# aslpavel/svgrasterize.py

Measured on AMD Instinct MI355X. Metric: Mpixels/sec AA coverage+composite (path-pixels/s; whole step: flatten+binning+coverage+composite; planned replay -- a frame with new geometry: value_replan), higher is better.
Workload: dtype f64 arithmetic, f32 RGBA store; 1 GPU; synthetic 4096 random closed cubic paths @ 4096x4096 (SURVEY 8d generator, splitmix64 0x5F3759DF); edges=783607

## Files before the change

### svgrasterize.py_amd/csrc/svgr_core.h

```cpp
#pragma once
#include <math.h>
#include <stdint.h>

#if defined(__HIPCC__)
#define SVGR_HD __host__ __device__ __forceinline__
#define SVGR_UNROLL _Pragma("unroll")
#else
#define SVGR_HD static inline
#define SVGR_UNROLL
#endif

namespace svgr {

constexpr int kMaxFlattenDepth = 40;
constexpr double kZeroCut = 1e-6;

SVGR_HD void xform_point(const double* m6, double p0, double p1, double& o0, double& o1) {
    o0 = fma(p1, m6[1], p0 * m6[0]) + m6[2];
    o1 = fma(p1, m6[4], p0 * m6[3]) + m6[5];
}

SVGR_HD double dot4(double w0, double w1, double w2, double w3, double x0, double x1, double x2, double x3) {
    return fma(w0, x0, w2 * x2) + fma(w1, x1, w3 * x3);
}
// ... 262 lines not shown
            if (!put(x1i - 1, d * (1.0 - a2 - am))) return;
        }
        put(x1i, d * am);
    }
}

struct RowPieces {
    int x0i, n;
    double v[5];
};

SVGR_HD RowPieces row_record(double x, double x_next, double d) {
    RowPieces r;
    double x0 = x < x_next ? x : x_next;
    double x1 = x < x_next ? x_next : x;
    double x0_floor = floor(x0);
    r.x0i = clamp_to_int(x0_floor);
    double x1_ceil = ceil(x1);
    int x1i = clamp_to_int(x1_ceil);
    r.v[2] = r.v[3] = r.v[4] = 0.0;
    if (x1i <= r.x0i + 1) {
        double xmf = 0.5 * (x + x_next) - x0_floor;
        r.n = 1;
        r.v[0] = d * (1 - xmf);
        r.v[1] = d * xmf;
    } else {
        double s = 1 / (x1 - x0);
        double x0f = x0 - x0_floor;
        double x1f = x1 - x1_ceil + 1.0;
        double o = 1 - x0f;
        double a0 = 0.5 * s * (o * o);
        double am = 0.5 * s * (x1f * x1f);
        r.n = x1i - r.x0i;
        r.v[0] = d * a0;
        r.v[4] = d * am;
        if (r.n == 2) {
            r.v[1] = d * (1.0 - a0 - am);
        } else {
            double a1 = s * (1.5 - x0f);
            r.v[1] = d * (a1 - a0);
            r.v[2] = d * s;
            double a2 = a1 + (double)(x1i - r.x0i - 3) * s;
            r.v[3] = d * (1.0 - a2 - am);
        }
    }
    return r;
}

SVGR_HD int band_room(double x_in, double x_out, int nr, int cols, int px, int& lo, int& hi) {
    double xlo = x_in < x_out ? x_in : x_out, xhi = x_in < x_out ? x_out : x_in;
    xlo -= 1e-9 * (1.0 + fabs(xlo));
    xhi += 1e-9 * (1.0 + fabs(xhi));
    lo = clamp_to_int(floor(xlo));
    hi = clamp_to_int(floor(xhi));
    const int lo_c = lo > -1 ? lo : -1;
    int hi_c = hi > -1 ? hi : -1;
    hi_c = hi_c < cols ? hi_c : cols;
    const int nc = hi_c - lo_c, fold = lo < 0 ? 3 * nr : 0;
    int room = 2 * nr + nc;
    room = room < 6 * nr + nc / px + 1 ? room : 6 * nr + nc / px + 1;
    return (room < 13 * nr ? room : 13 * nr) + fold;
}

template <class Put>
SVGR_HD void apply_record(int x0i, int n, const double* v, Put&& put) {
    if (!put(x0i, v[0])) return;
    if (!put(x0i + 1, v[1])) return;
    if (n >= 3) {
        for (int xi = x0i + 2; xi < x0i + n - 1; ++xi)
            if (!put(xi, v[2])) return;
        if (!put(x0i + n - 1, v[3])) return;
    }
    if (n >= 2) put(x0i + n, v[4]);
}

SVGR_HD void row_span(double x, double x_next, int& lo, int& hi) {
    double x0 = x < x_next ? x : x_next;
    double x1 = x < x_next ? x_next : x;
    lo = clamp_to_int(floor(x0));
    int x1i = clamp_to_int(ceil(x1));
    hi = (x1i <= lo + 1) ? lo + 1 : x1i;
}

SVGR_HD double fill_nonzero_raw(double s) {
    double m = fabs(s);
    return m > 1.0 ? 1.0 : m;
}
SVGR_HD double fill_nonzero(double s) {
    double m = fill_nonzero_raw(s);
    return m < kZeroCut ? 0.0 : m;
}
SVGR_HD double fill_evenodd_raw(double s) {
    double a = s + 1.0;
    double r = a - 2.0 * floor(a * 0.5);
    return fabs(r - 1.0);
}
SVGR_HD double fill_evenodd(double s) {
    double a = s + 1.0;
    double r = a - 2.0 * floor(a * 0.5);
    double m = fabs(r - 1.0);
    return m < kZeroCut ? 0.0 : m;
}
SVGR_HD double fill_rule(double s, int rule) { return rule ? fill_evenodd(s) : fill_nonzero(s); }

SVGR_HD void over_px(double* dst, double s0, double s1, double s2, double s3) {
    double k = 1 - s3;
    dst[0] = s0 + dst[0] * k;
    dst[1] = s1 + dst[1] * k;
    dst[2] = s2 + dst[2] * k;
    dst[3] = s3 + dst[3] * k;
}

SVGR_HD void over_px_fma(double* dst, double s0, double s1, double s2, double s3) {
    double k = 1 - s3;
    dst[0] = fma(dst[0], k, s0);
    dst[1] = fma(dst[1], k, s1);
    dst[2] = fma(dst[2], k, s2);
    dst[3] = fma(dst[3], k, s3);
}

constexpr int kTurbBSize = 0x100, kTurbBM = 0xff, kTurbN = 0x1000;
constexpr int kTurbLattice = kTurbBSize + kTurbBSize + 2;
constexpr int kTurbMaxOctaves = 32;
constexpr int64_t kTurbM = 2147483647, kTurbA = 16807, kTurbQ = 127773, kTurbR = 2836;

SVGR_HD int64_t turb_setup_seed(int64_t s) {
    if (s <= 0) s = -(s % (kTurbM - 1)) + 1;
    if (s > kTurbM - 1) s = kTurbM - 1;
    return s;
}

SVGR_HD int64_t turb_random(int64_t s) {
    int64_t r = kTurbA * (s % kTurbQ) - kTurbR * (s / kTurbQ);
    if (r <= 0) r += kTurbM;
    return r;
}

SVGR_HD void turb_init(int64_t seed, int* sel, double* grad) {
    int64_t s = turb_setup_seed(seed);
    for (int k = 0; k < 4; ++k) {
        for (int i = 0; i < kTurbBSize; ++i) {
            sel[i] = i;
            for (int j = 0; j < 2; ++j) {
                s = turb_random(s);
                grad[(i * 4 + k) * 2 + j] = (double)(s % (2 * kTurbBSize) - kTurbBSize) / kTurbBSize;
            }
            double* g = grad + (i * 4 + k) * 2;
            const double len = sqrt(g[0] * g[0] + g[1] * g[1]);
            if (len > 0.0) {
                g[0] = g[0] / len;
                g[1] = g[1] / len;
            }
        }
    }
    for (int i = kTurbBSize - 1; i > 0; --i) {
        const int t = sel[i];
        s = turb_random(s);
        const int j = (int)(s % kTurbBSize);
        sel[i] = sel[j];
        sel[j] = t;
    }
    for (int i = 0; i < kTurbBSize + 2; ++i) {
        sel[kTurbBSize + i] = sel[i];
        for (int q = 0; q < 8; ++q) grad[(kTurbBSize + i) * 8 + q] = grad[i * 8 + q];
    }
}
// ... 482 lines not shown
```

### svgrasterize.py_amd/csrc/svgr_hip.hip

```cpp
#include <hip/hip_runtime.h>

#include <algorithm>
#include <atomic>
#include <cstdarg>
#include <cstddef>
#include <cmath>
#include <cstdio>
#include <cstring>
#include <ctime>
#include <initializer_list>
#include <new>
#include <string>
#include <type_traits>
#include <vector>
#include <memory>
#include <unordered_map>
#include <utility>

#include "../../include/svgr.h"
#include "svgr_core.h"

using namespace svgr;

static std::atomic<unsigned long long> g_n_launches{0};
#define SVGR_LAUNCH(...) do { g_n_launches.fetch_add(1, std::memory_order_relaxed); hipLaunchKernelGGL(__VA_ARGS__); } while (0)

constexpr int TR = 16;
constexpr int PX = 8;
constexpr int CH = 8;
constexpr int TC = CH * PX;
constexpr int NT = TR * CH;
constexpr int CHUNK_STRIDE = PX + 2;
constexpr int ROW_STRIDE = CH * CHUNK_STRIDE;
constexpr int DELTA_BYTES = TR * ROW_STRIDE * 8;
static_assert(DELTA_BYTES < (1 << 16), "a TileAdd carries its byte offset in 16 bits");
static_assert(TC <= 64, "a TileAdd carries its run length in 6 bits");
constexpr int NW = NT / 64;
constexpr int WAVES_PER_EU = 4;
static_assert(NT % 64 == 0 && NT <= 1024, "tile kernel: whole waves, at most 1024 threads");

struct TileAdd {
    unsigned where;
    unsigned zero;
    double v;
};
static_assert(sizeof(TileAdd) == 16, "TileAdd is one dwordx4");
__device__ __forceinline__ void store_add(TileAdd* p, unsigned where, double v) {
    TileAdd t;
    t.where = where; t.zero = 0u; t.v = v;
    *p = t;
}
struct CellHdr {
    double paint[4];
    int r0, c0, rows, cols;
    int bits;
    int n_add, add0;
    int p;
    int group, pad[3];
    double carry[TR];
};
constexpr int HDR_DWORDS = 20;
constexpr int HDR_LOAD_DWORDS = HDR_DWORDS + 2 * TR;
static_assert(HDR_LOAD_DWORDS <= 64, "a CellHdr is one dword per lane of one load instruction");
static_assert(sizeof(CellHdr) == 4 * HDR_DWORDS + 8 * TR && offsetof(CellHdr, carry) == 4 * HDR_DWORDS, "CellHdr layout");
constexpr unsigned SPAN_MAX = (1u << 26) - 1;
static_assert(TR <= 64, "row-in-band is stored in 6 bits");

static thread_local std::string g_err;
static int fail(int code, const char* fmt, ...) {
    char buf[512];
    va_list ap;
    va_start(ap, fmt);
    vsnprintf(buf, sizeof buf, fmt, ap);
    va_end(ap);
    g_err = buf;
    return code;
}
#define HIPCHK(expr)                                                                              \
    do {                                                                                          \
        hipError_t e_ = (expr);                                                                   \
        if (e_ != hipSuccess) return fail(SVGR_E_HIP, "%s: %s (%s:%d)", #expr, hipGetErrorString(e_), __FILE__, __LINE__); \
    } while (0)

struct svgr_ctx {
    int device = 0;
    int id = 0;
    hipStream_t stream = nullptr;
    bool own_stream = false;
    char name[128] = {0};
    void* pinned = nullptr;
    size_t pinned_bytes = 0;
    void* up_stage = nullptr;
    size_t up_stage_bytes = 0;
    hipEvent_t up_ev = nullptr;
    bool up_busy = false;
    hipEvent_t meas_ev[2] = {nullptr, nullptr};
    hipEvent_t pin_ev = nullptr;
    struct WorkSpare* spare = nullptr;
    int n_cu = 256;
    void* trash = nullptr;
    unsigned* tile_ctr = nullptr;
    int tile_ctr_set = 0;
    static constexpr int N_SIDE = 8;
    hipStream_t side[N_SIDE] = {};
    hipEvent_t side_ev[N_SIDE] = {};
    hipEvent_t fork_ev = nullptr;
    bool side_ready = false;
};
static thread_local int tl_ctx_id = 0;
static hipError_t enter_ctx(const svgr_ctx* c) {
    tl_ctx_id = c->id;
    return hipSetDevice(c->device);
}
struct svgr_buf {
    void* ptr = nullptr;
    size_t bytes = 0;
// ... 928 lines not shown
#pragma unroll
        for (int j = 0; j < 4; ++j) {
            const int p = p_wave + (g0 + j) * 64 + lane;
            mem[j] = g0 + j < groups && p < n_paths && tb[j].nb > 0 && band >= tb[j].b0 && band < tb[j].b0 + tb[j].nb;
        }
    };
    for (int g0 = BE_KEEP; g0 < groups; g0 += 4) {
        PathBin tb[4];
        int4 tbb[4];
        bool mem[4];
        load4(g0, tb, tbb, mem);
#pragma unroll
        for (int j = 0; j < 4; ++j)
            if (mem[j]) { ++my_n; my_c += ctiles_of(tbb[j]); }
    }
    int wn = my_n, wc = my_c;
#pragma unroll
    for (int d = 1; d < 64; d <<= 1) { wn += __shfl_xor(wn, d); wc += __shfl_xor(wc, d); }
    if (lane == 0) { s_n[wave] = wn; s_c[wave] = wc; }
    __syncthreads();
    if (wave == 0) {
        const int a = lane < NWV ? s_n[lane] : 0, cc = lane < NWV ? s_c[lane] : 0;
        int tn, tcc;
        const int ea = wave_excl_scan(a, lane, tn);
        (void)wave_excl_scan(cc, lane, tcc);
        if (lane < NWV) s_n[lane] = ea;
        if (lane == 0) {
            int e0, i0, ok = 1;
            if (reuse) {
                e0 = pre_e0; i0 = pre_i0;
                if (pre_tn != tn) { atomicOr(&bd->err, 4); ok = 0; tn = 0; }
            } else {
                e0 = tn ? atomicAdd(&bd->entry_cursor, tn) : 0;
                i0 = tcc ? atomicAdd(&bd->item_cursor, tcc) : 0;
            }
            if (ok && e0 + tn > entry_cap) { atomicOr(&bd->err, 4); ok = 0; tn = 0; }
            if (ok && (long long)i0 + tcc > (long long)item_cap) { atomicOr(&bd->err, 64); ok = 0; tn = 0; }
            if (tn && !reuse) atomicMax(&bd->max_band_entries, tn);
            s_ent0 = e0; s_ok = ok;
            band_start[band] = e0;
            band_count[band] = tn;
            band_item0[band] = i0;
        }
    }
    __syncthreads();
    if (!s_ok) return;
    int ent = s_ent0 + s_n[wave];
    auto place = [&](bool m) {
        int tn;
        const int my_ent = ent + wave_excl_scan(m ? 1 : 0, lane, tn);
        ent += tn;
        return my_ent;
    };
    auto store = [&](int p, int my_ent, const int4 bb, const PathBin pbin) {
        TileEntry e;
        e.p = p; e.c0 = bb.y; e.cols = bb.w; e.r0 = bb.x; e.rows = bb.z;
        e.pad[0] = e.pad[1] = 0;
        int ct0, nct;
        path_ctiles(bb.y, bb.w, vc0, ct0, nct);
        e.cell0 = pbin.cell_off + (band - pbin.b0) * nct;
        entries[my_ent] = e;
        pair_idx[pbin.pb_off + band - pbin.b0] = my_ent - s_ent0;
    };
#pragma unroll
    for (int g = 0; g < BE_KEEP; ++g) {
        if (g >= groups) break;
        const int me = place(kmem[g]);
        if (kmem[g]) store(path_at(p_wave + g * 64 + lane), me, kbb[g], kb[g]);
    }
    for (int g0 = BE_KEEP; g0 < groups; g0 += 4) {
        PathBin tb[4];
        int4 tbb[4];
        bool mem[4];
        load4(g0, tb, tbb, mem);
#pragma unroll
        for (int j = 0; j < 4; ++j) {
            int me = 0;
            if (g0 + j < groups) me = place(mem[j]);
            if (mem[j]) store(path_at(p_wave + (g0 + j) * 64 + lane), me, tbb[j], tb[j]);
        }
    }
}

__device__ __forceinline__ double record_sum_range(int x0i, int n, const double* v, int ca, int cb) {
    auto in = [&](int xi) { const int c = xi > 0 ? xi : 0; return c >= ca && c < cb; };
    double sum = 0.0;
    if (in(x0i)) sum = v[0];
    if (in(x0i + 1)) sum = sum + v[1];
    if (n >= 3) {
        const int lo = ca > 0 ? (x0i + 2 > ca ? x0i + 2 : ca) : x0i + 2;
        const int hi = x0i + n - 2 < cb - 1 ? x0i + n - 2 : cb - 1;
        if (hi >= lo) sum = sum + (double)(hi - lo + 1) * v[2];
        if (in(x0i + n - 1)) sum = sum + v[3];
    }
    if (n >= 2 && in(x0i + n)) sum = sum + v[4];
    return sum;
}

template <class Single, class Run>
__device__ __forceinline__ void record_adds(int x0i, int n, const double* v, int ca, int cb, Single&& single, Run&& run) {
    auto one = [&](int xi, double val) {
        const int c = xi > 0 ? xi : 0;
        if (c >= ca && c < cb) single(c, val);
    };
    one(x0i, v[0]);
    one(x0i + 1, v[1]);
    if (n >= 3) {
        const int xa = x0i + 2, xb = x0i + n - 2;
        if (xa < 0 && ca == 0) {
            const int neg = (xb < -1 ? xb : -1) - xa + 1;
            if (neg > 0) single(0, (double)neg * v[2]);
        }
        int lo = xa > 0 ? xa : 0;
        lo = lo > ca ? lo : ca;
        const int hi = xb < cb - 1 ? xb : cb - 1;
        if (hi >= lo) run(lo, hi - lo + 1, v[2]);
        one(x0i + n - 1, v[3]);
    }
    if (n >= 2) one(x0i + n, v[4]);
}

__device__ __forceinline__ bool carry_visible(double c, int rule) {
    return (rule ? fill_evenodd_raw(c) : fabs(c)) >= kZeroCut;
}

__device__ __forceinline__ int lds_col(int tcol) {
    static_assert((PX & (PX - 1)) == 0, "PX is a power of two");
    return tcol + (int)((unsigned)tcol / PX) * (CHUNK_STRIDE - PX);
}
__device__ __forceinline__ int lds_index(int trow, int tcol) {
    return __mul24(trow, ROW_STRIDE) + lds_col(tcol);
}
__device__ __forceinline__ int run_pieces(int tcol, int len) {
    return ((tcol + len - 1) / PX) - (tcol / PX) + 1;
}
__device__ __forceinline__ unsigned add_where(int trow, int tcol, int len) {
    return (unsigned)(lds_index(trow, tcol) * 8) | ((unsigned)(len - 1) << 16) | ((unsigned)(tcol & (PX - 1)) << 22);
}

struct EdgeLds {
    double p0y, p1y, dxdy, x;
};
__device__ __forceinline__ double replay_rows(double x, int y, int n, double p0y, double p1y, double dxdy) {
    if (n <= 0) return x;
    RowState st;
    st.x_next = x; st.x = x; st.d = 0.0;
    row_step(st, y, p0y, p1y, dxdy, 1.0);
    double xn = st.x_next;
    for (int k = 1; k < n; ++k) xn = xn + dxdy;
    return xn;
}
static_assert(sizeof(EdgeLds) == 32, "EdgeLds is two 16-byte LDS reads (its first row and direction ride in an int array beside it)");
constexpr int PB_BATCH = 256;
constexpr int PB_EPL = (PB_BATCH + PB_THREADS - 1) / PB_THREADS;
static_assert(PB_BATCH % 64 == 0 && PB_BATCH / 16 <= 32, "two-level search: at most 32 coarse entries, read four at a time");
static_assert(PB_BANDS * TR * PB_BATCH < (1 << 20) && PB_BATCH < (1 << 11), "stage() scans row counts and live flags in one packed word");
constexpr int PB_WAVES = 6;
__device__ __forceinline__ void pb_barrier() { asm volatile("s_waitcnt lgkmcnt(0)\n\ts_barrier" ::: "memory"); }
template <int MODE>
__global__ __launch_bounds__(PB_THREADS, PB_WAVES) void k_path_build(const Slab* __restrict__ slabs, const double* __restrict__ edges,
                                                           const int* __restrict__ pair_idx, const double* __restrict__ path_paint,
                                                           const uint8_t* __restrict__ path_rule, const int* __restrict__ path_group,
                                                           const int* __restrict__ path_grad, int vr0, int vc0, int n_ct, int mask_words,
                                                           unsigned long long* __restrict__ tile_mask, CellHdr* __restrict__ cell_hdr,
                                                           int cell_cap, const AddShards ash, TileAdd* __restrict__ adds,
                                                           int2* __restrict__ cell_plan, BatchDev* __restrict__ bd, Owner own, int stats, int det,
                                                           unsigned long long* __restrict__ dbg,
                                                           const unsigned long long* __restrict__ guard_keys, const int* __restrict__ guard_bbox,
                                                           const PathBin* __restrict__ guard_bins, int n_paths, int vrows, int vcols) {
#ifdef SVGR_DBG_PB_STAMP
#define PB_STAMP(i) do { if (threadIdx.x == 0 && dbg && blockIdx.x < 8192) dbg[8 * blockIdx.x + (i)] = __builtin_amdgcn_s_memrealtime(); } while (0)
#else
#define PB_STAMP(i) do { } while (0)
#endif
    constexpr bool PLANNED = MODE != 0;
    constexpr bool BOUNDED = MODE == 2;
    PB_STAMP(0);
    __shared__ __attribute__((aligned(16))) double s_sum[PB_CELLS * TR];
    __shared__ double s_left[TR];
    __shared__ int s_cnt[PB_CELLS], s_pos[PB_CELLS], s_plan_n[PB_CELLS];
    __shared__ unsigned s_rowb[PB_CELLS + 1];
    __shared__ __attribute__((aligned(16))) EdgeLds s_edge[PB_BATCH];
    __shared__ int s_eya[PB_BATCH];
    __shared__ __attribute__((aligned(16))) int s_pref[PB_BATCH + 4];
    __shared__ unsigned short s_start[PB_THREADS];
    __shared__ int s_wtot[PB_EPL][PB_THREADS / 64];
    __shared__ __attribute__((aligned(8))) int2 s_info[PB_CELLS];
    __shared__ unsigned s_rowm[PB_CELLS];
    __shared__ int s_ptot[PB_BANDS], s_pidx[PB_BANDS], s_base, s_ok;
    const int tid = threadIdx.x, lane = tid & 63, wave = tid >> 6;
    for (int i = tid; i < PB_CELLS * TR / 2; i += PB_THREADS) ((double2*)s_sum)[i] = make_double2(0.0, 0.0);
    for (int i = tid; i < PB_CELLS; i += PB_THREADS) {
        s_cnt[i] = 0; s_pos[i] = (int)0x80000000; s_plan_n[i] = 0; s_rowb[i] = 0u; s_info[i] = make_int2(0, 0);
    }
    if (tid < TR) s_left[tid] = 0.0;
    if (tid == 0) s_rowb[PB_CELLS] = 0u;
    const Slab sl = slabs[blockIdx.x];
    const bool guarding = MODE == 1 && guard_keys != nullptr;
    const int n_slabs_now = guarding ? (int)gridDim.x : bd->slab_cursor;
    if ((int)blockIdx.x >= n_slabs_now) return;
    if (sl.nb <= 0 || sl.nk <= 0) return;
    PB_STAMP(7);
    const int p = sl.p;
    const int r0 = sl.r0, c0 = sl.c0, rows = sl.rows, cols = sl.cols;
    int ct0, nct;
    path_ctiles(c0, cols, vc0, ct0, nct);
    const int x_first = vc0 + ct0 * TC - c0;
    const int e_begin = sl.e_begin, e_end = sl.e_end;
    const int sr0 = vr0 + sl.band0 * TR - r0, sr1 = sr0 + sl.nb * TR;
    const int n_cell = sl.nb * sl.nk;
    const double o_r = (double)r0, o_c = (double)c0;
    const int rl = path_rule[p], rule = rl & 1;
    const int group = path_group ? path_group[p] : -1;
    const int grad1 = path_grad ? path_grad[p] + 1 : 0;
    const double4 paint = ((const double4*)path_paint)[p];
    auto cell_of = [&](int g, int k) { return sl.cell_off + (sl.band0 + g - sl.b0) * nct + sl.k0 + k; };
    int s_per = 0;
    int2 my_plan = make_int2((int)0x80000000, 0);
    bool plan_pending = false;
    int my_pidx = 0;
    if ((tid & (TR - 1)) == 0 && tid / TR < sl.nb && owns_band(own, sl.band0 + tid / TR)) my_pidx = pair_idx[sl.pb_off + sl.band0 + tid / TR - sl.b0];
    if (PLANNED && !BOUNDED) {
        if (tid < n_cell) {
            const int g = tid / sl.nk, k = tid - g * sl.nk;
            const int cell = cell_of(g, k);
            if (cell < cell_cap) my_plan = cell_plan[cell];
        }
        plan_pending = true;
    }

    auto stage = [&](int eb, bool bounds = false) -> int {
        int cnt[PB_EPL], eya[PB_EPL];
        EdgeLds el[PB_EPL];
#pragma unroll
        for (int j = 0; j < PB_EPL; ++j) {
            const int e = eb + tid + j * PB_THREADS;
            cnt[j] = 0;
            el[j].p0y = el[j].p1y = el[j].dxdy = el[j].x = 0.0; eya[j] = 0;
            if (e < e_end && tid + j * PB_THREADS < PB_BATCH) {
                const double4 ed = ((const double4*)edges)[e];
                const double ar = ed.x - o_r, ac = ed.y - o_c, br = ed.z - o_r, bc = ed.w - o_c;
                const EdgeSetup es = edge_setup(ar, ac, br, bc, rows);
                const double cmin = ac < bc ? ac : bc;
                if (es.valid && !(cmin >= (double)cols + 2.0)) {
                    const int ya = es.y_begin > sr0 ? es.y_begin : sr0, yb = es.y_end < sr1 ? es.y_end : sr1;
                    if (ya < yb) {
                        cnt[j] = yb - ya;
                        el[j].p0y = es.p0y; el[j].p1y = es.p1y; el[j].dxdy = es.dxdy; el[j].x = replay_rows(es.x, es.y_begin, ya - es.y_begin, es.p0y, es.p1y, es.dxdy);
                        eya[j] = ya | (es.dir < 0.0 ? (int)0x80000000 : 0);
                    }
                }
            }
        }
#ifdef SVGR_DBG_PB_STAMP
        if (PLANNED && eb == e_begin) { asm volatile("s_waitcnt vmcnt(0)" ::: "memory"); PB_STAMP(5); }
#endif
        int excl[PB_EPL], wtot[PB_EPL];
#pragma unroll
        for (int j = 0; j < PB_EPL; ++j) excl[j] = wave_excl_scan(cnt[j] | ((cnt[j] > 0 ? 1 : 0) << 20), lane, wtot[j]);
        pb_barrier();
        if (PLANNED && plan_pending) {
            if (tid < PB_CELLS) { s_pos[tid] = my_plan.x; s_plan_n[tid] = my_plan.y; }
            plan_pending = false;
        }
        if (BOUNDED && bounds) {
#pragma unroll
            for (int j = 0; j < PB_EPL; ++j) {
                if (cnt[j] <= 0) continue;
                const int ya = eya[j] & 0x7fffffff, yb = ya + cnt[j];
                const double dx = el[j].dxdy;
                const double ylo = (double)ya > el[j].p0y ? (double)ya : el[j].p0y;
                for (int y0 = ya; y0 < yb;) {
                    const int vrow = r0 + y0 - vr0, band = vrow / TR;
                    int y1 = y0 + TR - (vrow & (TR - 1));
                    y1 = y1 < yb ? y1 : yb;
                    if (owns_band(own, band)) {
                        const double ta = ((double)y0 > el[j].p0y ? (double)y0 : el[j].p0y) - ylo;
                        const double tb = ((double)y1 < el[j].p1y ? (double)y1 : el[j].p1y) - ylo;
                        int lo, hi;
                        const int room = band_room(el[j].x + dx * ta, el[j].x + dx * tb, y1 - y0, cols, PX, lo, hi);
                        if (lo < cols) {
                            const int cf = lo > 0 ? lo : 0;
                            int cl = hi + 1 > 0 ? hi + 1 : 0;
                            cl = cl < cols - 1 ? cl : cols - 1;
                            int kf = (cf - x_first) / TC, kl = (cl - x_first) / TC;
                            kf = kf > sl.k0 ? kf : sl.k0;
                            kl = kl < sl.k0 + sl.nk - 1 ? kl : sl.k0 + sl.nk - 1;
                            for (int k = kf; k <= kl; ++k)
                                __hip_atomic_fetch_add(&s_plan_n[(band - sl.band0) * sl.nk + (k - sl.k0)], room, __ATOMIC_RELAXED, __HIP_MEMORY_SCOPE_WORKGROUP);
                        }
                    }
                    y0 = y1;
                }
            }
        }
#pragma unroll
        for (int j = 0; j < PB_EPL; ++j)
            if (lane == 0) s_wtot[j][wave] = wtot[j];
        pb_barrier();
        int all = 0;
        int pre[PB_EPL];
#pragma unroll
        for (int j = 0; j < PB_EPL; ++j) {
            int before = all;
#pragma unroll
            for (int w = 0; w < PB_THREADS / 64; ++w) { before += w < wave ? s_wtot[j][w] : 0; all += s_wtot[j][w]; }
            pre[j] = before + excl[j];
        }
        const int n_live = all >> 20, total = all & 0xfffff;
        const int nl = det ? 64 : PB_THREADS;
        const int per = (total + nl - 1) / nl;
        s_per = per;
        const float inv_per = per > 0 ? 1.0f / (float)per : 0.f;
#pragma unroll
        for (int j = 0; j < PB_EPL; ++j) {
            if (cnt[j] > 0) {
                const int cs = pre[j] >> 20, tp = pre[j] & 0xfffff;
                s_edge[cs] = el[j];
                s_eya[cs] = eya[j];
                s_pref[cs] = tp;
                if (cs == n_live - 1) s_pref[n_live] = 0x7fffffff;
                int k0 = (int)((float)tp * inv_per);
                k0 += k0 * per < tp ? 1 : 0;
                k0 -= (k0 - 1) * per >= tp ? 1 : 0;
                for (int k = k0; k * per < tp + cnt[j]; ++k) s_start[k] = (unsigned short)cs;
            }
        }
        pb_barrier();
        return total;
    };
    struct RowAt {
        int x0i, n;
        double v[5];
        int where;
    };
    auto row_at = [&](double x, double x_next, double d, int y) -> RowAt {
        RowAt ra;
        const RowPieces rp = row_record(x, x_next, d);
        ra.x0i = rp.x0i; ra.n = rp.n;
        ra.v[0] = rp.v[0]; ra.v[1] = rp.v[1]; ra.v[2] = rp.v[2]; ra.v[3] = rp.v[3]; ra.v[4] = rp.v[4];
        if ((unsigned)ra.n > SPAN_MAX) { atomicOr(&bd->err, 16); ra.n = (int)SPAN_MAX; }
        const int vrow = r0 + y - vr0, band = vrow / TR;
        const bool live = owns_band(own, band) && rp.x0i < cols;
        ra.where = (band - sl.band0) | ((vrow & (TR - 1)) << 8) | ((int)live << 16);
        return ra;
    };
    auto for_rows = [&](int total, auto&& body) {
        const int nl = det ? 64 : PB_THREADS;
        const int per = s_per;
        int t = tid * per;
        const int t1 = t + per < total ? t + per : total;
        if (tid >= nl || t >= t1) return;
        const int slot0 = s_start[tid];
        int slot = slot0;
        const int dy = t - s_pref[slot0];
        EdgeLds el = s_edge[slot];
        int ya_dir = s_eya[slot];
        int y = ya_dir & 0x7fffffff;
        double dir = ya_dir < 0 ? -1.0 : 1.0;
        int t_next = s_pref[slot + 1];
        RowState st;
        st.x_next = replay_rows(el.x, y, dy, el.p0y, el.p1y, el.dxdy);
        st.x = st.x_next; st.d = 0.0;
        y += dy;
        for (; t < t1; ++t, ++y) {
            if (t == t_next) {
                ++slot;
                el = s_edge[slot];
                ya_dir = s_eya[slot];
                y = ya_dir & 0x7fffffff;
                dir = ya_dir < 0 ? -1.0 : 1.0;
                t_next = s_pref[slot + 1];
                st.x_next = el.x;
            }
            row_step(st, y, el.p0y, el.p1y, el.dxdy, dir);
            body(row_at(st.x, st.x_next, st.d, y));
        }
    };
    auto row_tiles = [&](const RowAt& ra, int& kf, int& kl) {
        const int xl = ra.x0i + (ra.n >= 2 ? ra.n : 1);
        const int cf = ra.x0i > 0 ? ra.x0i : 0;
        int cl = xl > 0 ? xl : 0;
        cl = cl < cols - 1 ? cl : cols - 1;
        kf = (cf - x_first) / TC;
        kl = (cl - x_first) / TC;
        kl = kl < sl.k0 + sl.nk - 1 ? kl : sl.k0 + sl.nk - 1;
    };
    auto tile_cols = [&](int k, int& ca, int& cb) {
        ca = k * TC + x_first;
        cb = ca + TC;
        ca = ca > 0 ? ca : 0;
        cb = cb < cols ? cb : cols;
    };
    auto store_pieces = [&](const RowAt& ra, int trow, int ca, int cb, int cell_c0, TileAdd* dst) {
        record_adds(ra.x0i, ra.n, ra.v, ca, cb,
                    [&](int c, double val) { store_add(dst++, add_where(trow, c - cell_c0, 1), val); },
                    [&](int c, int len, double val) {
                        int tc = c - cell_c0;
                        while (len > 0) {
                            const int n = len < PX - (tc & (PX - 1)) ? len : PX - (tc & (PX - 1));
                            store_add(dst++, add_where(trow, tc, n), val);
                            tc += n; len -= n;
                        }
                    });
    };
    auto count_row = [&](const RowAt& ra, auto store) {
        constexpr bool STORE = decltype(store)::value;
        if (!((ra.where >> 16) & 1)) return;
        const int bl = ra.where & 0xff, trow = (ra.where >> 8) & 0xff;
        int kf, kl;
        row_tiles(ra, kf, kl);
        if (sl.k0 > 0 && kf < sl.k0) {
            int ca, cb;
            tile_cols(sl.k0, ca, cb);
            const double part = record_sum_range(ra.x0i, ra.n, ra.v, 0, ca);
            __hip_atomic_fetch_add(&s_left[trow], part, __ATOMIC_RELAXED, __HIP_MEMORY_SCOPE_WORKGROUP);
            __hip_atomic_fetch_or(&s_rowb[PB_CELLS], 1u << trow, __ATOMIC_RELAXED, __HIP_MEMORY_SCOPE_WORKGROUP);
            kf = sl.k0;
        }
        for (int k = kf; k <= kl; ++k) {
            int ca, cb;
            tile_cols(k, ca, cb);
            int ne = 0;
            double part = 0.0;
            const int cell_c0 = k * TC + x_first;
            record_adds(ra.x0i, ra.n, ra.v, ca, cb, [&](int, double val) { ++ne; part = part + val; },
                        [&](int c, int len, double val) { ne += run_pieces(c - cell_c0, len); part = part + (double)len * val; });
            if (ne == 0) continue;
            const int ci = bl * sl.nk + (k - sl.k0);
            const int pos = __hip_atomic_fetch_add(&s_cnt[ci], ne, __ATOMIC_RELAXED, __HIP_MEMORY_SCOPE_WORKGROUP);
            __hip_atomic_fetch_add(&s_sum[ci * TR + trow], part, __ATOMIC_RELAXED, __HIP_MEMORY_SCOPE_WORKGROUP);
            __hip_atomic_fetch_or(&s_rowb[ci], 1u << trow, __ATOMIC_RELAXED, __HIP_MEMORY_SCOPE_WORKGROUP);
            if (STORE) {
                const int first = s_pos[ci];
                if (first < 0 || pos + ne > s_plan_n[ci]) continue;
                store_pieces(ra, trow, ca, cb, cell_c0, adds + ((size_t)first + pos));
            }
        }
    };
    auto emit_row = [&](const RowAt& ra) {
        if (!((ra.where >> 16) & 1)) return;
        const int bl = ra.where & 0xff, trow = (ra.where >> 8) & 0xff;
        int kf, kl;
        row_tiles(ra, kf, kl);
        kf = kf > sl.k0 ? kf : sl.k0;
        for (int k = kf; k <= kl; ++k) {
            int ca, cb;
            tile_cols(k, ca, cb);
            int ne = 0;
            const int cell_c0 = k * TC + x_first;
            record_adds(ra.x0i, ra.n, ra.v, ca, cb, [&](int, double) { ++ne; },
                        [&](int c, int len, double) { ne += run_pieces(c - cell_c0, len); });
            if (ne == 0) continue;
            const int ci = bl * sl.nk + (k - sl.k0);
            const int pos = __hip_atomic_fetch_add(&s_pos[ci], ne, __ATOMIC_RELAXED, __HIP_MEMORY_SCOPE_WORKGROUP);
            if (pos < 0) continue;
            store_pieces(ra, trow, ca, cb, cell_c0, adds + pos);
        }
    };

    const bool one_batch = e_end - e_begin <= PB_BATCH;
    int total = 0, n_rows = 0;
    if (BOUNDED) {
        for (int eb = e_begin; eb < e_end; eb += PB_BATCH) {
            total = stage(eb, true);
            n_rows += total;
        }
        PB_STAMP(1);
        static_assert(PB_CELLS <= 128, "the cells' places: a prefix sum by the first two waves");
        int room = 0, excl = 0;
        if (tid < 128) {
            const int bnd = tid < n_cell ? s_plan_n[tid] : 0;
            const int gg = tid < n_cell ? tid / sl.nk : 0, kk = tid < n_cell ? tid - gg * sl.nk : 0;
            const bool ends_here = cols - ((sl.k0 + kk) * TC + x_first) < TC;
            const int b_lo = vr0 + (sl.band0 + gg) * TR - r0;
            const int rin = (b_lo + TR < rows ? b_lo + TR : rows) - (b_lo > 0 ? b_lo : 0);
            room = bnd > 0 ? bnd + rin + (ends_here ? rin : 0) : 0;
            int wt;
            excl = wave_excl_scan(room, lane, wt);
            if (lane == 0) s_ptot[wave] = wt;
        }
        pb_barrier();
        if (tid == 0) {
            const int all = s_ptot[0] + s_ptot[1];
            const int sh = p % ash.n;
            int at = 0;
            if (all > 0) at = atomicAdd(&bd->shard[sh].add_cursor, all);
            int ok = 1;
            if ((long long)at + all > (long long)ash.cap[sh]) { atomicOr(&bd->err, 64); ok = 0; }
            s_base = ash.base[sh] + at;
            s_ok = ok;
        }
        pb_barrier();
        if (tid < n_cell) s_pos[tid] = room > 0 && s_ok ? s_base + (wave ? s_ptot[0] : 0) + excl : (int)0x80000000;
        pb_barrier();
        if (one_batch) {
            for_rows(total, [&](const RowAt& ra) { count_row(ra, std::true_type{}); });
        } else {
            for (int eb = e_begin; eb < e_end; eb += PB_BATCH) {
                const int tot = stage(eb);
                for_rows(tot, [&](const RowAt& ra) { count_row(ra, std::true_type{}); });
            }
        }
    } else
    for (int eb = e_begin; eb < e_end; eb += PB_BATCH) {
        total = stage(eb);
        PB_STAMP(1);
        n_rows += total;
        if (PLANNED) for_rows(total, [&](const RowAt& ra) { count_row(ra, std::true_type{}); });
        else for_rows(total, [&](const RowAt& ra) { count_row(ra, std::false_type{}); });
    }
    if (stats && tid == 0 && n_rows > 0) atomicAdd(&bd->bseg_cursor, n_rows);
    if (guarding && __builtin_amdgcn_readfirstlane(wave) == 0) {
        const int grid = (int)gridDim.x, g0 = ((int)blockIdx.x + grid - grid / 2) % grid;
        for (int g = g0; g * 64 < n_paths; g += grid) {
            const int q = g * 64 + lane;
            if (q >= n_paths) continue;
            const unsigned long long* k = guard_keys + 4 * (size_t)q;
            const int4 bb = ((const int4*)guard_bbox)[q];
            const PathBox pb = path_box(k[0], k[1], k[2], k[3], 1, vr0, vc0, vrows, vcols, TR, TC);
            if (pb.refused) atomicOr(&bd->err, 16);
            if (!path_box_is(pb, bb.x, bb.y, bb.z, bb.w, guard_bins[q].nb)) atomicOr(&bd->err, 32);
        }
    }
    pb_barrier();
    PB_STAMP(2);
    auto write_cell = [&](int g, int k, int cls, double cin, unsigned cm, unsigned sm, int own_n, int n_list, int add0, int row_l, int idx,
                          bool slab_ok) -> bool {
        const int band = sl.band0 + g;
        const int cell = cell_of(g, k);
        const bool mask_ok = (unsigned)(idx >> 6) < (unsigned)mask_words;
        if (!(cell < cell_cap && slab_ok && mask_ok) || (PLANNED && cls == 2 && add0 < 0)) {
            if (row_l == 0) atomicOr(&bd->err, 32);
            return false;
        }
        CellHdr* hd = cell_hdr + cell;
        if (cls == 1) hd->carry[row_l] = cin;
        const int cell_c0 = (sl.k0 + k) * TC + x_first;
        const unsigned below = (1u << row_l) - 1u;
        const int n_carry = __popc(cm);
        if (((cm >> row_l) & 1u) && adds) {
            store_add(adds + ((size_t)add0 + own_n + __popc(cm & below)), add_where(row_l, cell_c0 < 0 ? -cell_c0 : 0, 1), cin);
        }
        if (((sm >> row_l) & 1u) && adds) {
            store_add(adds + ((size_t)add0 + own_n + n_carry + __popc(sm & below)), add_where(row_l, cols - cell_c0, 1), __builtin_nan(""));
        }
        if (row_l == 0) {
            unsigned long long* const mw = tile_mask + ((size_t)band * n_ct + ct0 + sl.k0 + k) * 2 * mask_words + (idx >> 6);
            const unsigned long long mbit = 1ull << (idx & 63);
            atomicOr(mw, mbit);
            if (cls == 2) atomicOr(mw + mask_words, mbit);
            hd->paint[0] = paint.x; hd->paint[1] = paint.y; hd->paint[2] = paint.z; hd->paint[3] = paint.w;
            hd->r0 = r0; hd->c0 = c0; hd->rows = rows; hd->cols = cols;
            hd->bits = rule | (((rl >> 1) & 3) << 1) | (cls << 3) | (grad1 << 5);
            hd->n_add = n_list; hd->add0 = add0; hd->p = p;
            hd->group = group;
        }
        return true;
    };
    {
        static_assert(TR <= 16, "k_path_build packs two TR-bit row masks into one word");
        constexpr unsigned long long GMASK = (1ull << TR) - 1ull;
        const int g = tid / TR, row_l = tid & (TR - 1);
        const int shift = lane & ~(TR - 1);
        const int band = sl.band0 + g;
        const bool active = g < sl.nb && owns_band(own, band);
        const int row_abs = vr0 + band * TR + row_l;
        const bool row_in_layer = row_abs >= r0 && row_abs < r0 + rows;
        int cursor = 0;
        bool mismatch = false;
        if (__ballot(active) != 0ull) {
            const int idx = my_pidx;
            if (!PLANNED && active && row_l == 0) s_pidx[g] = idx;
            double run = sl.k0 > 0 ? s_left[row_l] : 0.0;
            unsigned had = sl.k0 > 0 ? s_rowb[PB_CELLS] : 0u;
            const unsigned sent_rows = (unsigned)((__ballot(active && row_in_layer) >> shift) & GMASK);
            for (int k = 0; k < sl.nk; ++k) {
                const int ci = g * sl.nk + k;
                const int own_n = active ? s_cnt[ci] : 0;
                const double sq = active ? s_sum[ci * TR + row_l] : 0.0;
                const unsigned rb = active ? s_rowb[ci] : 0u;
                const double cin = run;
                const bool vis = active && carry_visible(cin, rule);
                const unsigned long long vm = (__ballot(vis) >> shift) & GMASK;
                const int cls = own_n > 0 ? 2 : (vm != 0ull ? 1 : 0);
                const int t_end = cols - ((sl.k0 + k) * TC + x_first);
                const unsigned cm = cls == 2 ? had & (unsigned)GMASK : 0u;
                const unsigned sm = cls == 2 && t_end < TC ? sent_rows : 0u;
                const int n_add = cls == 2 ? __popc(cm) + __popc(sm) + own_n : 0;
                if (active) {
                    if (PLANNED) {
                        if (row_l == 0 && (BOUNDED ? own_n > s_plan_n[ci] : own_n != s_plan_n[ci])) mismatch = true;
                        if (BOUNDED && row_l == 0) {
                            const int cell = cell_of(g, k);
                            if (cell < cell_cap) cell_plan[cell] = make_int2(cls == 2 ? s_pos[ci] : (int)0x80000000, cls == 2 ? own_n : 0);
                        }
                        if (cls != 0) write_cell(g, k, cls, cin, cm, sm, own_n, n_add, s_pos[ci], row_l, idx, true);
                    } else {
                        s_sum[ci * TR + row_l] = cin;
                        if (row_l == 0) {
                            s_cnt[ci] = n_add;
                            s_info[ci] = make_int2(cursor, cls);
                            s_rowm[ci] = cm | (sm << 16);
                        }
                    }
                }
                cursor += n_add;
                run = run + sq;
                had |= rb;
            }
        }
        if (PLANNED) {
            if (mismatch) atomicOr(&bd->err, 32);
        } else {
            if (row_l == 0 && g < PB_BANDS) s_ptot[g] = active ? cursor : 0;
            pb_barrier();
            if (tid < 64) {
                static_assert(PB_BANDS <= 64, "one lane per band of the slab");
                const int c = tid < sl.nb ? s_ptot[tid] : 0;
                int all;
                const int ex = wave_excl_scan(c, tid, all);
                if (tid < sl.nb) s_ptot[tid] = ex;
                if (tid == 0) {
                    const int sh = p % ash.n;
                    int at = 0;
                    if (all > 0) at = atomicAdd(&bd->shard[sh].add_cursor, all);
                    int ok = 1;
                    if (adds && (long long)at + all > (long long)ash.cap[sh]) { atomicOr(&bd->err, 64); ok = 0; }
                    s_base = ash.base[sh] + at;
                    s_ok = ok;
                }
            }
            pb_barrier();
        }
    }
    PB_STAMP(3);
    if (!PLANNED) {
        const bool slab_ok = s_ok != 0;
        for (int i = tid; i < n_cell * TR; i += PB_THREADS) {
            const int ci = i / TR, row_l = i & (TR - 1);
            const int2 info = s_info[ci];
            const unsigned rowm = s_rowm[ci];
            const int cls = info.y & 3, g = ci / sl.nk, k = ci - g * sl.nk;
            if (!owns_band(own, sl.band0 + g)) continue;
            const int cell = cell_of(g, k);
            const int n_list = s_cnt[ci];
            const unsigned cm = rowm & 0xffffu, sm = rowm >> 16;
            const int own_n = n_list - __popc(cm) - __popc(sm);
            const int add0 = s_base + s_ptot[g] + info.x;
            if (row_l == 0 && cell < cell_cap) cell_plan[cell] = make_int2(cls == 2 && slab_ok ? add0 : (int)0x80000000, cls == 2 ? own_n : 0);
            if (cls == 0) continue;
            const bool ok = write_cell(g, k, cls, s_sum[i], cm, sm, own_n, n_list, add0, row_l, s_pidx[g], slab_ok);
            if (ok && row_l == 0 && cls == 2 && adds) s_pos[ci] = add0;
        }
    }
// ... 4817 lines not shown
```

Before: 804,000 Mpixels/s.

## Split planned path-build store pass and defer pair index load to LDS

Moves the record helpers into the shared core header and adds a separate store_row routine for the planned path. It counts and writes tile adds in one walk, with a fast branch for records that lie wholly inside a tile. In the planned mode the per-band pair index is loaded later, inside stage, and handed through LDS rather than held in a register across the kernel. Empty asm barriers pin some values to scalar or vector registers. The aim is to cut register pressure and redundant recounting in k_path_build, at the cost of more code paths and a small extra LDS round trip.

```diff
diff --git a/svgrasterize.py_amd/csrc/svgr_core.h b/svgrasterize.py_amd/csrc/svgr_core.h
--- a/svgrasterize.py_amd/csrc/svgr_core.h
+++ b/svgrasterize.py_amd/csrc/svgr_core.h
@@ -368,6 +368,133 @@
     hi = (x1i <= lo + 1) ? lo + 1 : x1i;
 }
 
+constexpr int kTilePX = 8;
+constexpr int kTileCH = 8;
+constexpr int kTileTC = kTileCH * kTilePX;
+constexpr int kChunkStride = kTilePX + 2;
+constexpr int kRowStride = kTileCH * kChunkStride;
+
+SVGR_HD double record_sum_range(int x0i, int n, const double* v, int ca, int cb) {
+    auto in = [&](int xi) { const int c = xi > 0 ? xi : 0; return c >= ca && c < cb; };
+    double sum = 0.0;
+    if (in(x0i)) sum = v[0];
+    if (in(x0i + 1)) sum = sum + v[1];
+    if (n >= 3) {
+        const int lo = ca > 0 ? (x0i + 2 > ca ? x0i + 2 : ca) : x0i + 2;
+        const int hi = x0i + n - 2 < cb - 1 ? x0i + n - 2 : cb - 1;
+        if (hi >= lo) sum = sum + (double)(hi - lo + 1) * v[2];
+        if (in(x0i + n - 1)) sum = sum + v[3];
+    }
+    if (n >= 2 && in(x0i + n)) sum = sum + v[4];
+    return sum;
+}
+
+template <class Single, class Run>
+SVGR_HD void record_adds(int x0i, int n, const double* v, int ca, int cb, Single&& single, Run&& run) {
+    auto one = [&](int xi, double val) {
+        const int c = xi > 0 ? xi : 0;
+        if (c >= ca && c < cb) single(c, val);
+    };
+    one(x0i, v[0]);
+    one(x0i + 1, v[1]);
+    if (n >= 3) {
+        const int xa = x0i + 2, xb = x0i + n - 2;
+        if (xa < 0 && ca == 0) {
+            const int neg = (xb < -1 ? xb : -1) - xa + 1;
+            if (neg > 0) single(0, (double)neg * v[2]);
+        }
+        int lo = xa > 0 ? xa : 0;
+        lo = lo > ca ? lo : ca;
+        const int hi = xb < cb - 1 ? xb : cb - 1;
+        if (hi >= lo) run(lo, hi - lo + 1, v[2]);
+        one(x0i + n - 1, v[3]);
+    }
+    if (n >= 2) one(x0i + n, v[4]);
+}
+
+SVGR_HD int lds_col(int tcol) {
+    static_assert((kTilePX & (kTilePX - 1)) == 0, "kTilePX is a power of two");
+    return tcol + (int)((unsigned)tcol / kTilePX) * (kChunkStride - kTilePX);
+}
+SVGR_HD int run_pieces(int tcol, int len) {
+    return ((tcol + len - 1) / kTilePX) - (tcol / kTilePX) + 1;
+}
+SVGR_HD unsigned add_where(int trow, int tcol, int len) {
+    return (unsigned)((trow * kRowStride + lds_col(tcol)) * 8) | ((unsigned)(len - 1) << 16) | ((unsigned)(tcol & (kTilePX - 1)) << 22);
+}
+
+SVGR_HD int record_count(int x0i, int n, int ca, int cb, int cell_c0) {
+    auto in = [&](int xi) { const int c = xi > 0 ? xi : 0; return c >= ca && c < cb ? 1 : 0; };
+    int ne = in(x0i) + in(x0i + 1);
+    if (n >= 3) {
+        const int xa = x0i + 2, xb = x0i + n - 2;
+        if (xa < 0 && ca == 0 && (xb < -1 ? xb : -1) - xa + 1 > 0) ++ne;
+        int lo = xa > 0 ? xa : 0;
+        lo = lo > ca ? lo : ca;
+        const int hi = xb < cb - 1 ? xb : cb - 1;
+        if (hi >= lo) ne += run_pieces(lo - cell_c0, hi - lo + 1);
+        ne += in(x0i + n - 1);
+    }
+    if (n >= 2) ne += in(x0i + n);
+    return ne;
+}
+template <bool PUT, class Put>
+SVGR_HD double record_walk(int x0i, int n, const double* v, int ca, int cb, int cell_c0, Put&& put) {
+    double part = 0.0;
+    record_adds(x0i, n, v, ca, cb,
+                [&](int c, double val) {
+                    part = part + val;
+                    if (PUT) put(c - cell_c0, 1, val);
+                },
+                [&](int c, int len, double val) {
+                    part = part + (double)len * val;
+                    if (PUT) {
+                        int tc = c - cell_c0;
+                        while (len > 0) {
+                            const int m = len < kTilePX - (tc & (kTilePX - 1)) ? len : kTilePX - (tc & (kTilePX - 1));
+                            put(tc, m, val);
+                            tc += m; len -= m;
+                        }
+                    }
+                });
+    return part;
+}
+SVGR_HD bool record_whole(int x0i, int n, int ca, int cb) {
+    return x0i >= ca && x0i + (n >= 2 ? n : 1) < cb;
+}
+SVGR_HD int record_count_whole(int tcol, int n) {
+    return n >= 4 ? 4 + run_pieces(tcol + 2, n - 3) : (n >= 2 ? n + 1 : 2);
+}
+template <bool PUT, class Put>
+SVGR_HD double record_walk_whole(int tcol, int n, const double* v, Put&& put) {
+    double part = 0.0;
+    part = part + v[0];
+    if (PUT) put(tcol, 1, v[0]);
+    part = part + v[1];
+    if (PUT) put(tcol + 1, 1, v[1]);
+    if (n >= 3) {
+        int len = n - 3;
+        if (len > 0) {
+            part = part + (double)len * v[2];
+            if (PUT) {
+                int tc = tcol + 2;
+                while (len > 0) {
+                    const int m = len < kTilePX - (tc & (kTilePX - 1)) ? len : kTilePX - (tc & (kTilePX - 1));
+                    put(tc, m, v[2]);
+                    tc += m; len -= m;
+                }
+            }
+        }
+        part = part + v[3];
+        if (PUT) put(tcol + n - 1, 1, v[3]);
+    }
+    if (n >= 2) {
+        part = part + v[4];
+        if (PUT) put(tcol + n, 1, v[4]);
+    }
+    return part;
+}
+
 SVGR_HD double fill_nonzero_raw(double s) {
     double m = fabs(s);
     return m > 1.0 ? 1.0 : m;
diff --git a/svgrasterize.py_amd/csrc/svgr_hip.hip b/svgrasterize.py_amd/csrc/svgr_hip.hip
--- a/svgrasterize.py_amd/csrc/svgr_hip.hip
+++ b/svgrasterize.py_amd/csrc/svgr_hip.hip
@@ -26,12 +26,12 @@
 #define SVGR_LAUNCH(...) do { g_n_launches.fetch_add(1, std::memory_order_relaxed); hipLaunchKernelGGL(__VA_ARGS__); } while (0)
 
 constexpr int TR = 16;
-constexpr int PX = 8;
-constexpr int CH = 8;
-constexpr int TC = CH * PX;
+constexpr int PX = kTilePX;
+constexpr int CH = kTileCH;
+constexpr int TC = kTileTC;
 constexpr int NT = TR * CH;
-constexpr int CHUNK_STRIDE = PX + 2;
-constexpr int ROW_STRIDE = CH * CHUNK_STRIDE;
+constexpr int CHUNK_STRIDE = kChunkStride;
+constexpr int ROW_STRIDE = kRowStride;
 constexpr int DELTA_BYTES = TR * ROW_STRIDE * 8;
 static_assert(DELTA_BYTES < (1 << 16), "a TileAdd carries its byte offset in 16 bits");
 static_assert(TC <= 64, "a TileAdd carries its run length in 6 bits");
@@ -1126,60 +1126,12 @@
     }
 }
 
-__device__ __forceinline__ double record_sum_range(int x0i, int n, const double* v, int ca, int cb) {
-    auto in = [&](int xi) { const int c = xi > 0 ? xi : 0; return c >= ca && c < cb; };
-    double sum = 0.0;
-    if (in(x0i)) sum = v[0];
-    if (in(x0i + 1)) sum = sum + v[1];
-    if (n >= 3) {
-        const int lo = ca > 0 ? (x0i + 2 > ca ? x0i + 2 : ca) : x0i + 2;
-        const int hi = x0i + n - 2 < cb - 1 ? x0i + n - 2 : cb - 1;
-        if (hi >= lo) sum = sum + (double)(hi - lo + 1) * v[2];
-        if (in(x0i + n - 1)) sum = sum + v[3];
-    }
-    if (n >= 2 && in(x0i + n)) sum = sum + v[4];
-    return sum;
-}
-
-template <class Single, class Run>
-__device__ __forceinline__ void record_adds(int x0i, int n, const double* v, int ca, int cb, Single&& single, Run&& run) {
-    auto one = [&](int xi, double val) {
-        const int c = xi > 0 ? xi : 0;
-        if (c >= ca && c < cb) single(c, val);
-    };
-    one(x0i, v[0]);
-    one(x0i + 1, v[1]);
-    if (n >= 3) {
-        const int xa = x0i + 2, xb = x0i + n - 2;
-        if (xa < 0 && ca == 0) {
-            const int neg = (xb < -1 ? xb : -1) - xa + 1;
-            if (neg > 0) single(0, (double)neg * v[2]);
-        }
-        int lo = xa > 0 ? xa : 0;
-        lo = lo > ca ? lo : ca;
-        const int hi = xb < cb - 1 ? xb : cb - 1;
-        if (hi >= lo) run(lo, hi - lo + 1, v[2]);
-        one(x0i + n - 1, v[3]);
-    }
-    if (n >= 2) one(x0i + n, v[4]);
-}
-
 __device__ __forceinline__ bool carry_visible(double c, int rule) {
     return (rule ? fill_evenodd_raw(c) : fabs(c)) >= kZeroCut;
 }
 
-__device__ __forceinline__ int lds_col(int tcol) {
-    static_assert((PX & (PX - 1)) == 0, "PX is a power of two");
-    return tcol + (int)((unsigned)tcol / PX) * (CHUNK_STRIDE - PX);
-}
 __device__ __forceinline__ int lds_index(int trow, int tcol) {
     return __mul24(trow, ROW_STRIDE) + lds_col(tcol);
-}
-__device__ __forceinline__ int run_pieces(int tcol, int len) {
-    return ((tcol + len - 1) / PX) - (tcol / PX) + 1;
-}
-__device__ __forceinline__ unsigned add_where(int trow, int tcol, int len) {
-    return (unsigned)(lds_index(trow, tcol) * 8) | ((unsigned)(len - 1) << 16) | ((unsigned)(tcol & (PX - 1)) << 22);
 }
 
 struct EdgeLds {
@@ -1198,6 +1150,7 @@
 constexpr int PB_BATCH = 256;
 constexpr int PB_EPL = (PB_BATCH + PB_THREADS - 1) / PB_THREADS;
 static_assert(PB_BATCH % 64 == 0 && PB_BATCH / 16 <= 32, "two-level search: at most 32 coarse entries, read four at a time");
+static_assert(PB_THREADS / TR <= PB_BANDS, "k_path_build keeps one word per TR-lane group in s_pidx");
 static_assert(PB_BANDS * TR * PB_BATCH < (1 << 20) && PB_BATCH < (1 << 11), "stage() scans row counts and live flags in one packed word");
 constexpr int PB_WAVES = 6;
 __device__ __forceinline__ void pb_barrier() { asm volatile("s_waitcnt lgkmcnt(0)\n\ts_barrier" ::: "memory"); }
@@ -1253,7 +1206,6 @@
     const int e_begin = sl.e_begin, e_end = sl.e_end;
     const int sr0 = vr0 + sl.band0 * TR - r0, sr1 = sr0 + sl.nb * TR;
     const int n_cell = sl.nb * sl.nk;
-    const double o_r = (double)r0, o_c = (double)c0;
     const int rl = path_rule[p], rule = rl & 1;
     const int group = path_group ? path_group[p] : -1;
     const int grad1 = path_grad ? path_grad[p] + 1 : 0;
@@ -1261,9 +1213,14 @@
     auto cell_of = [&](int g, int k) { return sl.cell_off + (sl.band0 + g - sl.b0) * nct + sl.k0 + k; };
     int s_per = 0;
     int2 my_plan = make_int2((int)0x80000000, 0);
-    bool plan_pending = false;
+    bool plan_pending = false, pidx_pending = PLANNED;
     int my_pidx = 0;
-    if ((tid & (TR - 1)) == 0 && tid / TR < sl.nb && owns_band(own, sl.band0 + tid / TR)) my_pidx = pair_idx[sl.pb_off + sl.band0 + tid / TR - sl.b0];
+    auto load_pidx = [&]() {
+        int t = tid;
+        asm volatile("" : "+v"(t));
+        return (t & (TR - 1)) == 0 && t / TR < sl.nb && owns_band(own, sl.band0 + t / TR) ? pair_idx[sl.pb_off + sl.band0 + t / TR - sl.b0] : 0;
+    };
+    if (!PLANNED) my_pidx = load_pidx();
     if (PLANNED && !BOUNDED) {
         if (tid < n_cell) {
             const int g = tid / sl.nk, k = tid - g * sl.nk;
@@ -1276,6 +1233,9 @@
     auto stage = [&](int eb, bool bounds = false) -> int {
         int cnt[PB_EPL], eya[PB_EPL];
         EdgeLds el[PB_EPL];
+        int r0_s = r0, c0_s = c0, cols_s = cols;
+        asm volatile("" : "+s"(r0_s), "+s"(c0_s), "+s"(cols_s));
+        const double o_r = (double)r0_s, o_c = (double)c0_s, c_beyond = (double)cols_s + 2.0;
 #pragma unroll
         for (int j = 0; j < PB_EPL; ++j) {
             const int e = eb + tid + j * PB_THREADS;
@@ -1286,7 +1246,7 @@
                 const double ar = ed.x - o_r, ac = ed.y - o_c, br = ed.z - o_r, bc = ed.w - o_c;
                 const EdgeSetup es = edge_setup(ar, ac, br, bc, rows);
                 const double cmin = ac < bc ? ac : bc;
-                if (es.valid && !(cmin >= (double)cols + 2.0)) {
+                if (es.valid && !(cmin >= c_beyond)) {
                     const int ya = es.y_begin > sr0 ? es.y_begin : sr0, yb = es.y_end < sr1 ? es.y_end : sr1;
                     if (ya < yb) {
                         cnt[j] = yb - ya;
@@ -1299,12 +1259,15 @@
 #ifdef SVGR_DBG_PB_STAMP
         if (PLANNED && eb == e_begin) { asm volatile("s_waitcnt vmcnt(0)" ::: "memory"); PB_STAMP(5); }
 #endif
+        if (PLANNED && pidx_pending) my_pidx = load_pidx();
         int excl[PB_EPL], wtot[PB_EPL];
 #pragma unroll
         for (int j = 0; j < PB_EPL; ++j) excl[j] = wave_excl_scan(cnt[j] | ((cnt[j] > 0 ? 1 : 0) << 20), lane, wtot[j]);
         pb_barrier();
         if (PLANNED && plan_pending) {
-            if (tid < PB_CELLS) { s_pos[tid] = my_plan.x; s_plan_n[tid] = my_plan.y; }
+            int tid_p = tid;
+            asm volatile("" : "+v"(tid_p));
+            if (tid_p < PB_CELLS) { s_pos[tid_p] = my_plan.x; s_plan_n[tid_p] = my_plan.y; }
             plan_pending = false;
         }
         if (BOUNDED && bounds) {
@@ -1342,6 +1305,10 @@
         for (int j = 0; j < PB_EPL; ++j)
             if (lane == 0) s_wtot[j][wave] = wtot[j];
         pb_barrier();
+        if (PLANNED && pidx_pending) {
+            if ((tid & (TR - 1)) == 0) s_pidx[tid / TR] = my_pidx;
+            pidx_pending = false;
+        }
         int all = 0;
         int pre[PB_EPL];
 #pragma unroll
@@ -1401,7 +1368,6 @@
         EdgeLds el = s_edge[slot];
         int ya_dir = s_eya[slot];
         int y = ya_dir & 0x7fffffff;
-        double dir = ya_dir < 0 ? -1.0 : 1.0;
         int t_next = s_pref[slot + 1];
         RowState st;
         st.x_next = replay_rows(el.x, y, dy, el.p0y, el.p1y, el.dxdy);
@@ -1413,11 +1379,10 @@
                 el = s_edge[slot];
                 ya_dir = s_eya[slot];
                 y = ya_dir & 0x7fffffff;
-                dir = ya_dir < 0 ? -1.0 : 1.0;
                 t_next = s_pref[slot + 1];
                 st.x_next = el.x;
             }
-            row_step(st, y, el.p0y, el.p1y, el.dxdy, dir);
+            row_step(st, y, el.p0y, el.p1y, el.dxdy, ya_dir < 0 ? -1.0 : 1.0);
             body(row_at(st.x, st.x_next, st.d, y));
         }
     };
@@ -1448,8 +1413,7 @@
                         }
                     });
     };
-    auto count_row = [&](const RowAt& ra, auto store) {
-        constexpr bool STORE = decltype(store)::value;
+    auto count_row = [&](const RowAt& ra) {
         if (!((ra.where >> 16) & 1)) return;
         const int bl = ra.where & 0xff, trow = (ra.where >> 8) & 0xff;
         int kf, kl;
@@ -1472,14 +1436,49 @@
                         [&](int c, int len, double val) { ne += run_pieces(c - cell_c0, len); part = part + (double)len * val; });
             if (ne == 0) continue;
             const int ci = bl * sl.nk + (k - sl.k0);
-            const int pos = __hip_atomic_fetch_add(&s_cnt[ci], ne, __ATOMIC_RELAXED, __HIP_MEMORY_SCOPE_WORKGROUP);
+            __hip_atomic_fetch_add(&s_cnt[ci], ne, __ATOMIC_RELAXED, __HIP_MEMORY_SCOPE_WORKGROUP);
             __hip_atomic_fetch_add(&s_sum[ci * TR + trow], part, __ATOMIC_RELAXED, __HIP_MEMORY_SCOPE_WORKGROUP);
             __hip_atomic_fetch_or(&s_rowb[ci], 1u << trow, __ATOMIC_RELAXED, __HIP_MEMORY_SCOPE_WORKGROUP);
-            if (STORE) {
-                const int first = s_pos[ci];
-                if (first < 0 || pos + ne > s_plan_n[ci]) continue;
-                store_pieces(ra, trow, ca, cb, cell_c0, adds + ((size_t)first + pos));
+        }
+    };
+    auto store_row = [&](const RowAt& ra) {
+        if (!((ra.where >> 16) & 1)) return;
+        const int bl = ra.where & 0xff, trow = (ra.where >> 8) & 0xff;
+        int kf, kl;
+        row_tiles(ra, kf, kl);
+        if (sl.k0 > 0 && kf < sl.k0) {
+            int ca, cb;
+            tile_cols(sl.k0, ca, cb);
+            const double part = record_sum_range(ra.x0i, ra.n, ra.v, 0, ca);
+            __hip_atomic_fetch_add(&s_left[trow], part, __ATOMIC_RELAXED, __HIP_MEMORY_SCOPE_WORKGROUP);
+            __hip_atomic_fetch_or(&s_rowb[PB_CELLS], 1u << trow, __ATOMIC_RELAXED, __HIP_MEMORY_SCOPE_WORKGROUP);
+            kf = sl.k0;
+        }
+        for (int k = kf; k <= kl; ++k) {
+            int ca, cb;
+            tile_cols(k, ca, cb);
+            const int cell_c0 = k * TC + x_first;
+            const bool whole = record_whole(ra.x0i, ra.n, ca, cb);
+            const int ne = whole ? record_count_whole(ra.x0i - cell_c0, ra.n) : record_count(ra.x0i, ra.n, ca, cb, cell_c0);
+            if (ne == 0) continue;
+            const int ci = bl * sl.nk + (k - sl.k0);
+            const int pos = __hip_atomic_fetch_add(&s_cnt[ci], ne, __ATOMIC_RELAXED, __HIP_MEMORY_SCOPE_WORKGROUP);
+            const int first = s_pos[ci];
+            const bool fits = !(first < 0 || pos + ne > s_plan_n[ci]);
+            TileAdd* dst = adds + ((size_t)first + pos);
+            auto put = [&](int tc, int len, double val) {
+                if (fits) store_add(dst, add_where(trow, tc, len), val);
+                ++dst;
+            };
+            double part;
+            if (whole) {
+                record_walk_whole<true>(ra.x0i - cell_c0, ra.n, ra.v, put);
+                part = record_walk_whole<false>(0, ra.n, ra.v, put);
+            } else {
+                part = record_walk<true>(ra.x0i, ra.n, ra.v, ca, cb, cell_c0, put);
             }
+            __hip_atomic_fetch_add(&s_sum[ci * TR + trow], part, __ATOMIC_RELAXED, __HIP_MEMORY_SCOPE_WORKGROUP);
+            __hip_atomic_fetch_or(&s_rowb[ci], 1u << trow, __ATOMIC_RELAXED, __HIP_MEMORY_SCOPE_WORKGROUP);
         }
     };
     auto emit_row = [&](const RowAt& ra) {
@@ -1539,11 +1538,11 @@
         if (tid < n_cell) s_pos[tid] = room > 0 && s_ok ? s_base + (wave ? s_ptot[0] : 0) + excl : (int)0x80000000;
         pb_barrier();
         if (one_batch) {
-            for_rows(total, [&](const RowAt& ra) { count_row(ra, std::true_type{}); });
+            for_rows(total, store_row);
         } else {
             for (int eb = e_begin; eb < e_end; eb += PB_BATCH) {
                 const int tot = stage(eb);
-                for_rows(tot, [&](const RowAt& ra) { count_row(ra, std::true_type{}); });
+                for_rows(tot, store_row);
             }
         }
     } else
@@ -1551,8 +1550,8 @@
         total = stage(eb);
         PB_STAMP(1);
         n_rows += total;
-        if (PLANNED) for_rows(total, [&](const RowAt& ra) { count_row(ra, std::true_type{}); });
-        else for_rows(total, [&](const RowAt& ra) { count_row(ra, std::false_type{}); });
+        if (PLANNED) for_rows(total, store_row);
+        else for_rows(total, count_row);
     }
     if (stats && tid == 0 && n_rows > 0) atomicAdd(&bd->bseg_cursor, n_rows);
     if (guarding && __builtin_amdgcn_readfirstlane(wave) == 0) {
@@ -1605,7 +1604,9 @@
     {
         static_assert(TR <= 16, "k_path_build packs two TR-bit row masks into one word");
         constexpr unsigned long long GMASK = (1ull << TR) - 1ull;
-        const int g = tid / TR, row_l = tid & (TR - 1);
+        int tid_w = tid;
+        asm volatile("" : "+v"(tid_w));
+        const int g = tid_w / TR, row_l = tid_w & (TR - 1);
         const int shift = lane & ~(TR - 1);
         const int band = sl.band0 + g;
         const bool active = g < sl.nb && owns_band(own, band);
@@ -1614,7 +1615,7 @@
         int cursor = 0;
         bool mismatch = false;
         if (__ballot(active) != 0ull) {
-            const int idx = my_pidx;
+            const int idx = PLANNED ? s_pidx[g < PB_BANDS ? g : 0] : my_pidx;
             if (!PLANNED && active && row_l == 0) s_pidx[g] = idx;
             double run = sl.k0 > 0 ? s_left[row_l] : 0.0;
             unsigned had = sl.k0 > 0 ? s_rowb[PB_CELLS] : 0u;
```

Measured after the change: 789,700 Mpixels/s. -1.8%, worse.
